# zhaoyuhsin/Edge-Guided-Near-Eye-Image-Analysis-for-Head-Mounted-Displays

Hardware: AMD Instinct MI355X
Metric: eye-frames/sec (320x240): inference edge+seg (value), +fit, exact fp32, and train fwd+bwd at 1 MI355X (higher is better)
Workload: dtype f32 tensors; inference products split into f16 hi/lo pairs (3 f16 MFMAs per product, 22-bit significand), f32 accumulate (`exact_fp32`: every product on the f32 MFMA); `train`: bf16 storage, f32 accumulate, f32 master weights (and an f32-storage leg)

## Files before the change

edge-guided-near-eye-image-analysis-for-head-mounted-displays_amd/_lib.py:

```python
import ctypes as C
import os

_HERE = os.path.dirname(os.path.abspath(__file__))
LIB_PATH = os.environ.get("EGNE_LIB") or os.path.join(_HERE, "csrc", "libegne_hip.so")

MAXSEG, MAXGROUP = 8, 3
ACT_NONE, ACT_RELU, ACT_LEAKY = 0, 1, 2

c_fp = C.c_void_p


class Seg(C.Structure):
    _fields_ = [("ptr", c_fp), ("pix_stride", C.c_int64), ("ch_off", C.c_int32), ("Cp", C.c_int32),
                ("scale", c_fp), ("shift", c_fp), ("act_in", C.c_int32), ("presplit", C.c_int32)]


class ConvDesc(C.Structure):
    _fields_ = [("B", C.c_int32), ("H", C.c_int32), ("W", C.c_int32), ("Ho", C.c_int32), ("Wo", C.c_int32),
                ("kh", C.c_int32), ("kw", C.c_int32), ("stride", C.c_int32),
                ("pad_h", C.c_int32), ("pad_w", C.c_int32), ("pad_mode", C.c_int32),
                ("ngroups", C.c_int32), ("dil", C.c_int32 * MAXGROUP),
                ("nseg", C.c_int32), ("seg", Seg * MAXSEG),
                ("Ktot", C.c_int32), ("CoutP", C.c_int32),
                ("w", c_fp), ("bias", c_fp), ("act", C.c_int32),
                ("post_scale", c_fp), ("post_shift", c_fp),
                ("residual", c_fp), ("res_pix_stride", C.c_int64), ("res_ch_off", C.c_int32),
                ("out", c_fp), ("out_pix_stride", C.c_int64), ("out_ch_off", C.c_int32),
                ("Cout_store", C.c_int32),
                ("stats_ws", c_fp), ("stats_nchunk", C.c_int32),
                ("pool_out", c_fp), ("pool_pix_stride", C.c_int64), ("pool_ch_off", C.c_int32),
                ("dyn_scale", C.c_void_p), ("absmax_out", C.c_void_p), ("dtype", C.c_int32),
                ("out_split", C.c_int32), ("out_split_scale", C.c_float), ("ovf_flag", C.c_void_p), ("f16_products", C.c_int32),
                ("mask_y", C.c_void_p), ("mask_pix_stride", C.c_int64), ("mask_ch_off", C.c_int32), ("mask_act", C.c_int32), ("mask_sums", C.c_void_p)]


class Dst(C.Structure):
    _fields_ = [("out", C.c_void_p), ("out_pix_stride", C.c_int64), ("out_ch_off", C.c_int32), ("C", C.c_int32), ("CoutP", C.c_int32),
                ("wfrag", C.c_void_p), ("residual", C.c_void_p), ("res_pix_stride", C.c_int64), ("res_ch_off", C.c_int32),
                ("mask_y", C.c_void_p), ("mask_pix_stride", C.c_int64), ("mask_ch_off", C.c_int32), ("act", C.c_int32),
                ("sums", C.c_void_p), ("res_pixels", C.c_int64)]


MAXDST = 6


class ConvQuery(C.Structure):
    _fields_ = [("dtype", C.c_int32), ("B", C.c_int32), ("H", C.c_int32), ("W", C.c_int32),
                ("kh", C.c_int32), ("kw", C.c_int32), ("stride", C.c_int32), ("pad_h", C.c_int32), ("pad_w", C.c_int32), ("pad_mode", C.c_int32),
                ("ngroups", C.c_int32), ("dil", C.c_int32 * MAXGROUP), ("nseg", C.c_int32),
                ("seg_C", C.c_int32 * MAXSEG), ("seg_Cp", C.c_int32 * MAXSEG), ("seg_ch_off", C.c_int32 * MAXSEG), ("seg_pix_stride", C.c_int64 * MAXSEG),
                ("seg_affine", C.c_int32 * MAXSEG), ("seg_planar", C.c_int32), ("seg_presplit", C.c_int32),
                ("Cout", C.c_int32), ("Cout_store", C.c_int32), ("dst_Cp", C.c_int32), ("dst_ch_off", C.c_int32), ("dst_pix_stride", C.c_int64),
                ("act", C.c_int32), ("has_post", C.c_int32), ("has_residual", C.c_int32), ("res_pix_stride", C.c_int64), ("res_ch_off", C.c_int32),
                ("split", C.c_int32), ("split1", C.c_int32), ("split_c4", C.c_int32), ("train", C.c_int32), ("dyn_scales", C.c_int32),
                ("is_dgrad", C.c_int32), ("want_stats", C.c_int32), ("want_pool", C.c_int32), ("pool_Cp", C.c_int32), ("pool_pix_stride", C.c_int64),
                ("want_scores", C.c_int32), ("up_add", C.c_int32), ("narrow_bf16_ok", C.c_int32), ("f16_products", C.c_int32), ("f16_storage", C.c_int32)]


class ConvChoice(C.Structure):
    _fields_ = [("kind", C.c_int32), ("name", C.c_char * 32), ("tail_frames", C.c_int32), ("fused_stats", C.c_int32), ("fused_pool", C.c_int32),
                ("small_ws_floats", C.c_int64)]


class BdcnTailDesc(C.Structure):
    _fields_ = [("B", C.c_int32), ("H", C.c_int32), ("W", C.c_int32),
                ("s", c_fp * 5), ("s1", c_fp * 5), ("h", C.c_int32 * 5), ("w", C.c_int32 * 5),
                ("stride", C.c_int32 * 5), ("crop", C.c_int32 * 5), ("up", c_fp * 5),
                ("fuse_w", c_fp), ("fuse_b", c_fp), ("out", c_fp * 11), ("edge_thres", C.c_int32)]


class LossDesc(C.Structure):
    _fields_ = [("B", C.c_int32), ("H", C.c_int32), ("W", C.c_int32),
                ("logits", c_fp), ("pix_stride", C.c_int64), ("ch_off", C.c_int32),
                ("target", c_fp), ("spatWts", c_fp), ("distMap", c_fp), ("cond", c_fp),
                ("pupil_center", c_fp), ("elNorm", c_fp), ("elOut", c_fp), ("alpha", C.c_float),
                ("grid_x", c_fp), ("grid_y", c_fp),
                ("partials", c_fp), ("out_terms", c_fp), ("pred_c", c_fp), ("elPred", c_fp),
                ("mask", c_fp), ("op_nchw", c_fp), ("coef", c_fp), ("dtype", C.c_int32),
                ("g_op_nchw", c_fp), ("g_pred_c", c_fp), ("g_elOut_up", c_fp)]


i32, i64, f32, vp = C.c_int32, C.c_int64, C.c_float, C.c_void_p
SIGNATURES = {
    "egne_conv2d_fwd": (i32, [C.POINTER(ConvDesc), vp]),
    "egne_pack_conv_weight": (i32, [vp, i32, i32, i32, i32, vp, i32, i32, vp, vp]),
    "egne_pack_conv_weight_frag": (i32, [vp, i32, i32, i32, i32, vp, i32, i32, vp, vp]),
    "egne_conv3x3_halo_supported": (i32, [C.POINTER(ConvDesc)]),
    "egne_conv3x3_halo_fwd": (i32, [C.POINTER(ConvDesc), vp]),
    "egne_conv3x3_smallcin_fwd": (i32, [C.POINTER(ConvDesc), vp, vp]),
    "egne_pack_conv_weight_f16x2": (i32, [vp, i32, i32, i32, i32, i32, i32, f32, vp, vp, vp]),
    "egne_conv2d_f16x3_fwd": (i32, [C.POINTER(ConvDesc), vp, vp, f32, f32, vp]),
    "egne_conv2d_f16x3_small_workspace_floats": (i64, [C.POINTER(ConvDesc)]),
    "egne_conv2d_f16x3_small_fwd": (i32, [C.POINTER(ConvDesc), vp, vp, f32, f32, vp, i64, vp]),
    "egne_pack_conv_weight_f16frag": (i32, [vp, i32, i32, i32, i32, i32, i32, f32, vp, vp, vp]),
    "egne_conv3x3_halo_f16_fwd": (i32, [C.POINTER(ConvDesc), vp, vp, f32, f32, vp]),
    "egne_conv1x1_3x3_fused_f16_fwd": (i32, [C.POINTER(ConvDesc), C.POINTER(ConvDesc), vp, vp, f32, f32, vp, vp, f32, f32, vp]),
    "egne_conv3x3c4_3x3_fused_f16_fwd": (i32, [C.POINTER(ConvDesc), C.POINTER(ConvDesc), vp, vp, f32, f32, vp, vp, f32, f32, vp]),
    "egne_msblock_dil_scores_f16_fwd": (i32, [C.POINTER(ConvDesc), vp, vp, f32, f32, vp, vp, vp, vp, i32, vp]),
    "egne_msblock_dil_f16_fwd": (i32, [C.POINTER(ConvDesc), vp, vp, f32, f32, vp]),
    "egne_conv3x3_rs_f16_fwd": (i32, [C.POINTER(ConvDesc), vp, vp, f32, f32, vp]),
    "egne_conv3x3_rw_f16_fwd": (i32, [C.POINTER(ConvDesc), vp, vp, f32, f32, vp]),
    "egne_conv1x1_pool2_f16x3_fwd": (i32, [C.POINTER(ConvDesc), vp, vp, f32, f32, vp]),
    "egne_conv1x1_f16x3_fwd": (i32, [C.POINTER(ConvDesc), vp, vp, f32, f32, vp]),
    "egne_dist_maps_workspace_bytes": (i64, [i32, i32, i32, i32]),
    "egne_dist_maps": (i32, [vp, i32, i32, i32, i32, vp, vp, vp]),
    "egne_zscore": (i32, [vp, vp, i32, i32, vp]),
    "egne_spatial_weights": (i32, [vp, i32, i32, i32, vp, vp]),
    "egne_eval_prep_workspace_bytes": (i64, [i32, i32, i32, i32, i32]),
    "egne_eval_prep": (i32, [vp, i32, i32, i32, i32, i32, i32, i32, vp, vp, vp, vp, i32, i32, vp, vp, vp, vp]),
    "egne_eval_render": (i32, [vp, i32, i32, i32, i32, i32, vp, vp, vp, i32, i32, C.c_double, i32, vp, vp, vp, vp, vp]),
    "egne_deepvog_loss_workspace_floats": (i64, [i32, i32, i32]),
    "egne_deepvog_loss_fwd": (i32, [vp, i64, i32, vp, vp, vp, i32, i32, i32, vp, vp, vp, vp, vp, vp]),
    "egne_deepvog_loss_bwd": (i32, [vp, i64, i32, vp, vp, vp, i32, i32, i32, vp, vp, vp, vp, i64, i32, vp]),
    "egne_affine_act": (i32, [vp, i64, i32, vp, i64, i32, i32, i64, vp, vp, i32, vp]),
    "egne_augment": (i32, [vp, vp, vp, vp, vp, vp, vp, vp, i32, i32, i32, vp]),
    "egne_augment_cv": (i32, [vp, vp, vp, vp, vp, vp, vp, vp, vp, vp, i32, i32, i32, vp]),
    "egne_conv3x3_smallcin_f16_fwd": (i32, [C.POINTER(ConvDesc), vp, vp, f32, f32, vp]),
    "egne_pack_conv3x3_c4_weight_f16": (i32, [vp, i32, i32, i32, f32, vp, vp, vp]),
    "egne_conv1x1_ms_f16x3_fwd": (i32, [C.POINTER(ConvDesc), vp, vp, f32, f32, vp]),
    "egne_pack_conv1x1_weight_f16x2_map": (i32, [vp, i32, i32, vp, i32, i32, f32, vp, vp, vp]),
    "egne_conv2d_f16x3_big_fwd": (i32, [C.POINTER(ConvDesc), vp, f32, f32, vp]),
    "egne_pack_conv_weight_f16img": (i32, [vp, i32, i32, i32, i32, i32, i32, f32, vp, vp]),
    "egne_conv2d_f16_big1_fwd": (i32, [C.POINTER(ConvDesc), vp, f32, f32, vp]),
    "egne_conv2d_f16_big1_supported": (i32, [C.POINTER(ConvDesc)]),
    "egne_pack_conv_weight_f16img1": (i32, [vp, i32, i32, i32, i32, i32, i32, f32, vp, vp]),
    "egne_pack_conv1x1_weight_f16": (i32, [vp, i32, i32, vp, i32, i32, f32, vp, vp, vp]),
    "egne_absmax": (i32, [vp, i64, i32, i32, i64, vp, vp]),
    "egne_absmax_f16": (i32, [vp, i64, i32, i32, i64, vp, vp]),
    "egne_norm_stats_workspace_bytes": (i64, [i32, i32, i32, i32]),
    "egne_norm_stats": (i32, [vp, i64, i32, i32, i32, i32, i32, f32, vp, vp, vp, vp, vp, vp]),
    "egne_norm_stats_finish": (i32, [vp, i32, i32, i32, i32, f32, vp, vp, vp]),
    "egne_norm_stats_finish_moments": (i32, [vp, i32, i32, i32, i32, f32, vp, vp, vp, vp, vp]),
    "egne_affine_inplace": (i32, [vp, i64, i32, i32, i64, vp, vp, vp]),
    "egne_affine": (i32, [vp, i64, i32, vp, i64, i32, i32, i64, vp, vp, vp]),
    "egne_avgpool2": (i32, [vp, i64, i32, vp, i64, i32, i32, i32, i32, i32, vp]),
    "egne_norm_act_pool2": (i32, [vp, i64, i32, vp, vp, i32, vp, i64, i32, i32, i32, i32, i32, vp]),
    "egne_maxpool2": (i32, [vp, i64, i32, vp, i64, i32, i32, i32, i32, i32, i32, i32, i32, vp]),
    "egne_maxpool2_f16": (i32, [vp, i64, i32, vp, i64, i32, i32, i32, i32, i32, i32, i32, i32, vp]),
    "egne_maxpool2_split": (i32, [vp, i64, i32, vp, i64, i32, i32, i32, i32, i32, i32, i32, i32, vp]),
    "egne_upsample2x": (i32, [vp, i64, i32, vp, i64, i32, i32, i32, i32, i32, vp]),
    "egne_upsample2x_nearest": (i32, [vp, i64, i32, vp, i64, i32, i32, i32, i32, i32, vp]),
    "egne_upsample2x_nearest_bwd": (i32, [vp, i64, i32, vp, i64, i32, i32, i32, i32, i32, vp]),
    "egne_nchw_to_nhwc": (i32, [vp, i32, i32, i32, i32, vp, i64, i32, i32, vp]),
    "egne_nhwc_to_nchw": (i32, [vp, i64, i32, i32, i32, i32, i32, vp, vp]),
    "egne_bdcn_stage_scores": (i32, [C.POINTER(vp), i32, i64, i64, vp, vp, vp, vp, vp, vp, vp, vp, vp]),
    "egne_bdcn_tail": (i32, [C.POINTER(BdcnTailDesc), vp]),
    "egne_loss_workspace_floats": (i64, [i32, i32, i32]),
    "egne_loss_fwd": (i32, [C.POINTER(LossDesc), vp]),
    "egne_ellipse_head_act": (i32, [vp, i32, i32, vp]),
    "egne_selu_inplace": (i32, [vp, i64, vp]),
    "egne_spatial_mean": (i32, [vp, i64, i32, i32, i32, i32, vp, vp]),
    "egne_softmax3": (i32, [vp, i64, i32, vp, i64, i32, i32, i64, vp]),
    "egne_adain": (i32, [vp, i64, i32, i32, vp, vp, i64, i32, vp, i64, i32, i32, i32, f32, vp]),
    "egne_conf_loss": (i32, [vp, i32, vp, i32, i32, i32, f32, vp, vp]),
    "egne_loss_bwd": (i32, [C.POINTER(LossDesc), vp, vp, i64, i32, vp, vp]),
    "egne_act_bwd_bias_workspace_bytes": (i64, [i64, i32]),
    "egne_act_bwd_bias": (i32, [vp, i64, i32, vp, i64, i32, i32, i32, i64, vp, i32, i32, vp, vp]),
    "egne_act_bwd_bias_absmax": (i32, [vp, i64, i32, vp, i64, i32, i32, i32, i64, vp, i32, i32, vp, vp, vp]),
    "egne_act_norm_bwd": (i32, [vp, i64, i32, vp, i64, i32, i32, vp, vp, vp, i64, i32, vp, i64, i32, i32, i32, i32, i32, i32, vp, vp, vp, i32, vp, i32, vp]),
    "egne_bn_act_bwd": (i32, [vp, i64, i32, i32, vp, vp, vp, vp, i64, i32, i32, i32, i32, i32, vp, i64, i32, vp, vp, vp, vp, i32, vp, i32, vp, vp]),
    "egne_zero_many": (i32, [vp, i32, i64, vp]),
    "egne_pair_bias_bwd_workspace_bytes": (i64, [i32, i32]),
    "egne_pair_bias_bwd": (i32, [vp, i64, i32, i32, i32, i32, i32, vp, vp, i32, i32, vp, vp, vp, vp]),
    "egne_norm_bwd_workspace_bytes": (i64, [i32, i32, i32, i32]),
    "egne_norm_pool2_bwd": (i32, [vp, i64, i32, vp, vp, vp, i64, i32, i32, i32, i32, i32, i32, vp, i64, i32, i32, vp, vp, vp]),
    "egne_norm_bwd_store": (i32, [vp, i64, i32, vp, vp, vp, vp, i64, i32, i32, i32, i32, i32, i32, vp, i64, i32, vp, vp, vp,
                                  i32, vp, vp]),
    "egne_norm_bwd": (i32, [vp, i64, i32, vp, vp, vp, vp, i64, i32, i32, i32, i32, i32, i32, vp, i64, i32, vp, vp, vp,
                            i32, vp, vp]),
    "egne_avgpool2_bwd": (i32, [vp, i64, i32, vp, i64, i32, i32, i32, i32, i32, vp]),
    "egne_upsample2x_bwd": (i32, [vp, i64, i32, vp, i64, i32, i32, i32, i32, i32, vp]),
    "egne_upsample2x_bwd_store": (i32, [vp, i64, i32, vp, i64, i32, i32, i32, i32, i32, vp]),
    "egne_ellipse_head_act_bwd": (i32, [vp, vp, i32, i32, vp]),
    "egne_selu_bwd": (i32, [vp, vp, i64, vp]),
    "egne_softmax3_bwd": (i32, [vp, i64, i32, vp, i64, i32, vp, i64, i32, i64, vp]),
    "egne_adain_bwd": (i32, [vp, i64, i32, i32, vp, i64, i32, vp, i64, i32, vp, i64, i32, vp, vp, i64, i32, i32, i32, f32, vp]),
    "egne_reflect_pad_bwd": (i32, [vp, i64, i32, i32, i32, vp, i64, i32, i32, i32, i32, i32, vp]),
    "egne_spatial_mean_bwd": (i32, [vp, i32, vp, i64, i32, i32, i32, i32, vp]),
    "egne_conf_loss_bwd": (i32, [vp, i32, vp, i32, i32, i32, vp, vp, i32, vp]),
    "egne_conv2d_wgrad_splits": (i32, [C.POINTER(ConvDesc)]),
    "egne_conv2d_wgrad_workspace_bytes": (i64, [C.POINTER(ConvDesc)]),
    "egne_conv2d_wgrad": (i32, [C.POINTER(ConvDesc), vp, i64, i32, i32, i32, vp, C.POINTER(vp), vp, vp]),
    "egne_conv2d_wgrad_f16": (i32, [C.POINTER(ConvDesc), vp, i64, i32, vp, i32, i32, vp, C.POINTER(vp), vp, vp]),
    "egne_pack_conv_weight_dgrad": (i32, [vp, i32, i32, i32, i32, i32, i32, i32, i32, i32, vp, vp]),
    "egne_ellipse_fit": (i32, [vp, i32, vp, vp, i32, i32, i32, vp, vp, vp, vp, vp, vp]),
    "egne_ellipse_init_from_pred": (i32, [vp, i32, i32, i32, vp, vp, vp, vp]),
# ... 63 lines not shown
```

edge-guided-near-eye-image-analysis-for-head-mounted-displays_amd/csrc/common.h:

```cpp
#pragma once
#include <hip/hip_runtime.h>
#include <cstdarg>
#include <cstdio>
#include <mutex>
#include <unordered_map>
#include "../../include/egne_hip.h"

static __device__ __attribute__((aligned(256), used)) float egne_zero_page[64] = {0};

typedef __bf16 egne_bf16;
typedef float egne_f32x4 __attribute__((ext_vector_type(4)));
typedef __bf16 egne_bf16x4 __attribute__((ext_vector_type(4)));
typedef __bf16 egne_bf16x8 __attribute__((ext_vector_type(8)));

__device__ __forceinline__ egne_f32x4 ld4(const float* p) { return *(const egne_f32x4*)p; }
__device__ __forceinline__ egne_f32x4 ld4(const egne_bf16* p) { return __builtin_convertvector(*(const egne_bf16x4*)p, egne_f32x4); }
__device__ __forceinline__ void st4(float* p, egne_f32x4 v) { *(egne_f32x4*)p = v; }
__device__ __forceinline__ void st4(egne_bf16* p, egne_f32x4 v) { *(egne_bf16x4*)p = __builtin_convertvector(v, egne_bf16x4); }
__device__ __forceinline__ float ld1(const float* p) { return *p; }
__device__ __forceinline__ float ld1(const egne_bf16* p) { return (float)*p; }
__device__ __forceinline__ void st1(float* p, float v) { *p = v; }
__device__ __forceinline__ void st1(egne_bf16* p, float v) { *p = (egne_bf16)v; }
template <typename T> struct egne_vt { static constexpr int N = 4; };
template <> struct egne_vt<egne_bf16> { static constexpr int N = 8; };
// ... 20 lines not shown
  *(egne_bf16x8*)p = egne_bf16x8{l[0], l[1], l[2], l[3], h[0], h[1], h[2], h[3]};
}
typedef unsigned egne_u32x4 __attribute__((ext_vector_type(4)));
template <typename T> __device__ __forceinline__ egne_u32x4 ldraw(const T* p) { return *(const egne_u32x4*)p; }
__device__ __forceinline__ egne_fv<4> unpackv(const float*, egne_u32x4 w) {
  return egne_fv<4>{{__builtin_bit_cast(float, w[0]), __builtin_bit_cast(float, w[1]), __builtin_bit_cast(float, w[2]), __builtin_bit_cast(float, w[3])}};
}
__device__ __forceinline__ egne_fv<8> unpackv(const egne_bf16*, egne_u32x4 w) {
  egne_fv<8> r;
#pragma unroll
  for (int i = 0; i < 4; ++i) {
    r.v[2 * i] = __builtin_bit_cast(float, w[i] << 16);
    r.v[2 * i + 1] = __builtin_bit_cast(float, w[i] & 0xffff0000u);
  }
  return r;
}
template <int N> __device__ __forceinline__ egne_fv<N> ldf(const float* p) {
  egne_fv<N> r;
#pragma unroll
  for (int i = 0; i < N; i += 4) { const egne_f32x4 t = *(const egne_f32x4*)(p + i); r.v[i] = t[0]; r.v[i + 1] = t[1]; r.v[i + 2] = t[2]; r.v[i + 3] = t[3]; }
  return r;
}
template <int N> __device__ __forceinline__ egne_fv<N> fv_fill(float x) {
  egne_fv<N> r;
#pragma unroll
  for (int i = 0; i < N; ++i) r.v[i] = x;
  return r;
}
template <typename T> __device__ __forceinline__ const T* zero_page() { return (const T*)egne_zero_page; }

#ifdef EGNE_NO_OVF_CHECK
__device__ __forceinline__ bool egne_nonfinite(float) { return false; }
__device__ __forceinline__ bool egne_nonfinite64(double) { return false; }
#else
__device__ __forceinline__ bool egne_nonfinite(float v) { return __builtin_amdgcn_classf(v, 0x207); }
__device__ __forceinline__ bool egne_nonfinite64(double v) { return !__builtin_isfinite(v); }
#endif
__device__ __forceinline__ bool egne_ovf_row(int y, int H) { return y % 3 == 1 || y == H - 1; }
__device__ __forceinline__ void egne_ovf_commit(bool bad, unsigned* flag) {
  if (flag && bad) atomicOr(flag, 1u);
}

namespace egne {

char* err_buf();

inline int fail(int code, const char* fmt, ...) {
  va_list ap;
  va_start(ap, fmt);
  vsnprintf(err_buf(), 512, fmt, ap);
  va_end(ap);
  return code;
}

inline bool fp32_storage(const egne_conv_desc& d) {
  for (int i = 0; i < d.nseg && i < EGNE_MAXSEG; ++i)
    if (d.seg[i].presplit != 0) return false;
  return d.out_split == 0;
}

inline int check_launch(const char* what) {
  hipError_t e = hipGetLastError();
  if (e != hipSuccess) return fail(EGNE_ERR_LAUNCH, "%s: %s", what, hipGetErrorString(e));
  return EGNE_OK;
}

inline bool raise_lds(const void* kern, size_t bytes) {
  static std::mutex mu;
  static std::unordered_map<const void*, size_t> have;
  std::lock_guard<std::mutex> g(mu);
  auto it = have.find(kern);
  if (it != have.end() && it->second >= bytes) return true;
  if (hipFuncSetAttribute(kern, hipFuncAttributeMaxDynamicSharedMemorySize, (int)bytes) != hipSuccess) {
    (void)hipGetLastError();
    return false;
  }
  have[kern] = bytes;
  return true;
}

#define EGNE_REQUIRE(cond, ...) \
  do { if (!(cond)) return ::egne::fail(EGNE_ERR_ARG, __VA_ARGS__); } while (0)

bool halo3_supported(const egne_conv_desc& d);
int halo3_launch(const egne_conv_desc& d, hipStream_t st);

bool wgrad_halo_supported(const egne_conv_desc& d, long long gzs);
int wgrad_halo_splits(const egne_conv_desc& d);
int wgrad_halo_launch(const egne_conv_desc& d, const float* gz, long long gzs, int gzo, float* ws, hipStream_t st);
int wgrad_halo_f16_launch(const egne_conv_desc& d, const float* gz, long long gzs, int gzo, const unsigned* gz_dyn, float* ws, hipStream_t st);

bool wgrad3x3_bf16_supported(const egne_conv_desc& d, long long gzs);
int wgrad3x3_bf16_splits(const egne_conv_desc& d);
int wgrad3x3_bf16_launch(const egne_conv_desc& d, const egne_bf16* gz, long long gzs, int gzo, float* ws, hipStream_t st);
bool wgrad1x1_bf16_supported(const egne_conv_desc& d, long long gzs);
int wgrad1x1_bf16_splits(const egne_conv_desc& d);
int wgrad1x1_bf16_launch(const egne_conv_desc& d, const egne_bf16* gz, long long gzs, int gzo, float* ws, hipStream_t st);

int msdil_ps_launch(const egne_conv_desc& d, const void* fhi, const void* flo, float a_scale, float w_scale, const float* score_w,
                    const float* score_c, float* s0, float* s1, int accumulate, hipStream_t st);

bool msdil1_wanted(const egne_conv_desc& d);
int msdil1_launch(const egne_conv_desc& d, const void* fhi, float a_scale, float w_scale, const float* score_w, const float* score_c,
                  float* s0, float* s1, int accumulate, hipStream_t st);

inline int cdiv(long long a, long long b) { return (int)((a + b - 1) / b); }

}
```

edge-guided-near-eye-image-analysis-for-head-mounted-displays_amd/csrc/conv1x1_f16.hip:

```cpp
#include "common.h"
#include "split_f16.h"

typedef float f32x16 __attribute__((ext_vector_type(16)));
typedef float f32x4 __attribute__((ext_vector_type(4)));
typedef float f32x2 __attribute__((ext_vector_type(2)));
typedef _Float16 h8 __attribute__((ext_vector_type(8)));
typedef _Float16 h2 __attribute__((ext_vector_type(2)));
typedef unsigned u32x4 __attribute__((ext_vector_type(4)));

namespace {

constexpr unsigned OOB = 0x80000000u;

__device__ __forceinline__ __amdgpu_buffer_rsrc_t make_rsrc(const void* base, unsigned bytes) {
  return __builtin_amdgcn_make_buffer_rsrc(const_cast<void*>(base), 0, (int)bytes, 0x00020000);
}

__device__ __forceinline__ void split8(const u32x4 a, const u32x4 b, float s, h8& hi, h8& lo) {
  const f32x4 va = __builtin_bit_cast(f32x4, a), vb = __builtin_bit_cast(f32x4, b);
  const float x[8] = {va[0], va[1], va[2], va[3], vb[0], vb[1], vb[2], vb[3]};
#pragma unroll
  for (int q = 0; q < 4; ++q) {
    h2 h, l;
    egne::split2(x[2 * q], x[2 * q + 1], s, h, l);
// ... 367 lines not shown
  EGNE_REQUIRE(lds <= 80 * 1024, "conv1x1_f16: K = %d groups of 16 does not fit the LDS weight image", G);
  static bool once = [] {
    return hipFuncSetAttribute((const void*)conv1x1_f16x3_kernel<1>, hipFuncAttributeMaxDynamicSharedMemorySize, 80 * 1024) == hipSuccess &&
           hipFuncSetAttribute((const void*)conv1x1_f16x3_kernel<2>, hipFuncAttributeMaxDynamicSharedMemorySize, 80 * 1024) == hipSuccess;
  }();
  if (!once) return egne::fail(EGNE_ERR_LAUNCH, "conv1x1_f16: cannot raise the dynamic LDS limit");
  const int ny = d.CoutP / (32 * TN);
  long long gx = (nb + 3) / 4;
  const long long cap = 256 * 8;
  if (gx > cap) gx = cap;
  const float os = 1.0f / (a_scale * w_scale);
  hipStream_t st = (hipStream_t)stream;
  if (up) {
    const size_t lds_up = lds + (size_t)4 * 18 * (32 * TN + 8) * sizeof(float);
    EGNE_REQUIRE(lds_up <= 80 * 1024, "conv1x1_f16: K = %d groups of 16 leaves no room for the addend patches", G);
    static bool once_up = [] {
      return hipFuncSetAttribute((const void*)conv1x1_f16x3_kernel<1, true>, hipFuncAttributeMaxDynamicSharedMemorySize, 80 * 1024) == hipSuccess &&
             hipFuncSetAttribute((const void*)conv1x1_f16x3_kernel<2, true>, hipFuncAttributeMaxDynamicSharedMemorySize, 80 * 1024) == hipSuccess;
    }();
    if (!once_up) return egne::fail(EGNE_ERR_LAUNCH, "conv1x1_f16: cannot raise the dynamic LDS limit");
    if (TN == 1)
      hipLaunchKernelGGL((conv1x1_f16x3_kernel<1, true>), dim3((unsigned)gx, ny), dim3(256), lds_up, st, d, (const _Float16*)fhi, (const _Float16*)flo,
                         a_scale, os, G, M, (int)nb);
    else
      hipLaunchKernelGGL((conv1x1_f16x3_kernel<2, true>), dim3((unsigned)gx, ny), dim3(256), lds_up, st, d, (const _Float16*)fhi, (const _Float16*)flo,
                         a_scale, os, G, M, (int)nb);
  } else if (TN == 1)
    hipLaunchKernelGGL((conv1x1_f16x3_kernel<1>), dim3((unsigned)gx, ny), dim3(256), lds, st, d, (const _Float16*)fhi, (const _Float16*)flo,
                       a_scale, os, G, M, (int)nb);
  else
    hipLaunchKernelGGL((conv1x1_f16x3_kernel<2>), dim3((unsigned)gx, ny), dim3(256), lds, st, d, (const _Float16*)fhi, (const _Float16*)flo,
                       a_scale, os, G, M, (int)nb);
  return egne::check_launch("egne_conv1x1_f16x3_fwd");
}

extern "C" int egne_conv1x1_pool2_f16x3_fwd(const egne_conv_desc* dp, const void* fhi, const void* flo, float a_scale, float w_scale,
                                            void* stream) {
  EGNE_REQUIRE(dp && fhi && flo, "conv1x1_pool2_f16: null pointer");
  const egne_conv_desc& d = *dp;
  EGNE_REQUIRE(egne::fp32_storage(d), "conv1x1_f16: split-pair / f16 storage (presplit, out_split) is not known here");
  EGNE_REQUIRE(d.kh == 1 && d.kw == 1 && d.stride == 1 && d.pad_h == 0 && d.pad_w == 0 && d.ngroups == 1 && d.Ho == d.H / 2 && d.Wo == d.W / 2 &&
               d.Ho > 0 && d.Wo > 0 && d.nseg >= 1 && d.nseg <= EGNE_MAXSEG && !d.residual && !d.post_scale, "conv1x1_pool2_f16: unsupported descriptor");
  EGNE_REQUIRE(d.CoutP % 32 == 0 && d.CoutP <= 96 && d.Cout_store <= d.CoutP && d.Cout_store % 4 == 0 && d.out &&
               ((uintptr_t)d.out & 15) == 0 && d.out_pix_stride % 4 == 0 && d.out_ch_off % 4 == 0 &&
               d.out_ch_off + d.Cout_store <= d.out_pix_stride && (!d.bias || ((uintptr_t)d.bias & 15) == 0), "conv1x1_pool2_f16: output");
  int G = 0;
  for (int s = 0; s < d.nseg; ++s) {
    const egne_seg& g = d.seg[s];
    EGNE_REQUIRE(g.ptr && g.scale && g.shift && ((uintptr_t)g.scale & 15) == 0 && ((uintptr_t)g.shift & 15) == 0 && g.Cp % 8 == 0 &&
                 g.ch_off % 4 == 0 && g.pix_stride % 4 == 0 && ((uintptr_t)g.ptr & 15) == 0 && g.ch_off + g.Cp <= g.pix_stride &&
                 (long long)d.H * d.W * g.pix_stride * 8 < (1ll << 31), "conv1x1_pool2_f16: slice %d", s);
    G += (g.Cp + 15) / 16;
  }
  EGNE_REQUIRE(d.out_pix_stride * 128 < (1ll << 31) && ((uintptr_t)fhi & 15) == 0 && ((uintptr_t)flo & 15) == 0 && a_scale > 0.f && w_scale > 0.f,
               "conv1x1_pool2_f16: strides / weights / scales");
  const long long M = (long long)d.B * d.Ho * d.Wo;
  const long long nb = (M + 31) / 32;
  EGNE_REQUIRE(nb < (1ll << 31), "conv1x1_pool2_f16: too many pixels");
  const int TN = d.CoutP / 32;
  const int bpf = (d.Ho * d.Wo + 31) / 32;
  EGNE_REQUIRE(!d.stats_ws || (((uintptr_t)d.stats_ws & 15) == 0 && d.stats_nchunk >= 1 && d.stats_nchunk <= bpf &&
                               (long long)(d.stats_nchunk - 1) * ((bpf + d.stats_nchunk - 1) / d.stats_nchunk) < bpf &&
                               (long long)d.B * d.stats_nchunk < (1ll << 31)),
               "conv1x1_pool2_f16: stats_ws needs 1 <= stats_nchunk <= %d blocks per frame, no empty chunk", bpf);
  const size_t lds = (size_t)G * TN * 2 * 64 * 8 * sizeof(_Float16) + (d.stats_ws ? (size_t)4 * 32 * 36 * sizeof(float) : 0);
  EGNE_REQUIRE(lds <= 80 * 1024, "conv1x1_pool2_f16: K = %d groups of 16 does not fit the LDS weight image", G);
  static bool once = [] {
    return hipFuncSetAttribute((const void*)conv1x1_pool_f16x3_kernel<1>, hipFuncAttributeMaxDynamicSharedMemorySize, 80 * 1024) == hipSuccess &&
           hipFuncSetAttribute((const void*)conv1x1_pool_f16x3_kernel<2>, hipFuncAttributeMaxDynamicSharedMemorySize, 80 * 1024) == hipSuccess &&
           hipFuncSetAttribute((const void*)conv1x1_pool_f16x3_kernel<3>, hipFuncAttributeMaxDynamicSharedMemorySize, 80 * 1024) == hipSuccess &&
           hipFuncSetAttribute((const void*)conv1x1_pool_f16x3_kernel<1, true>, hipFuncAttributeMaxDynamicSharedMemorySize, 80 * 1024) == hipSuccess &&
           hipFuncSetAttribute((const void*)conv1x1_pool_f16x3_kernel<2, true>, hipFuncAttributeMaxDynamicSharedMemorySize, 80 * 1024) == hipSuccess &&
           hipFuncSetAttribute((const void*)conv1x1_pool_f16x3_kernel<3, true>, hipFuncAttributeMaxDynamicSharedMemorySize, 80 * 1024) == hipSuccess;
  }();
  if (!once) return egne::fail(EGNE_ERR_LAUNCH, "conv1x1_pool2_f16: cannot raise the dynamic LDS limit");
  const int ny = 1;
  const long long nu = d.stats_ws ? (long long)d.B * d.stats_nchunk : nb;
  long long gx = (nu + 3) / 4;
  const long long cap = 256 * 8;
  if (gx > cap) gx = cap;
  const float os = 1.0f / (a_scale * w_scale);
  hipStream_t st = (hipStream_t)stream;
  const dim3 grid((unsigned)gx, (unsigned)ny);
  const _Float16* h = (const _Float16*)fhi;
  const _Float16* l = (const _Float16*)flo;
  if (d.stats_ws) {
    if (TN == 1) hipLaunchKernelGGL((conv1x1_pool_f16x3_kernel<1, true>), grid, dim3(256), lds, st, d, h, l, a_scale, os, G, M, (int)nu);
    else if (TN == 2) hipLaunchKernelGGL((conv1x1_pool_f16x3_kernel<2, true>), grid, dim3(256), lds, st, d, h, l, a_scale, os, G, M, (int)nu);
    else hipLaunchKernelGGL((conv1x1_pool_f16x3_kernel<3, true>), grid, dim3(256), lds, st, d, h, l, a_scale, os, G, M, (int)nu);
  } else if (TN == 1) hipLaunchKernelGGL((conv1x1_pool_f16x3_kernel<1>), grid, dim3(256), lds, st, d, h, l, a_scale, os, G, M, (int)nu);
  else if (TN == 2) hipLaunchKernelGGL((conv1x1_pool_f16x3_kernel<2>), grid, dim3(256), lds, st, d, h, l, a_scale, os, G, M, (int)nu);
  else hipLaunchKernelGGL((conv1x1_pool_f16x3_kernel<3>), grid, dim3(256), lds, st, d, h, l, a_scale, os, G, M, (int)nu);
  return egne::check_launch("egne_conv1x1_pool2_f16x3_fwd");
}
```

include/egne_hip.h:

```cpp
#ifndef EGNE_HIP_H
#define EGNE_HIP_H

#include <stdint.h>

#ifdef __cplusplus
extern "C" {
#endif

#define EGNE_MAXSEG 8
#define EGNE_MAXGROUP 3

typedef enum {
  EGNE_OK = 0,
  EGNE_ERR_ARG = -1,
  EGNE_ERR_LAUNCH = -2,
  EGNE_ERR_NODEVICE = -3
} egne_status;

typedef enum { EGNE_ACT_NONE = 0, EGNE_ACT_RELU = 1, EGNE_ACT_LEAKY = 2 } egne_act;

typedef struct {
  const float* ptr;
  int64_t pix_stride;
  int32_t ch_off;
// ... 1 lines not shown
  const float* scale;
  const float* shift;
  int32_t act_in;
  int32_t presplit;
} egne_seg;

typedef struct {
  int32_t B, H, W;
  int32_t Ho, Wo;
  int32_t kh, kw, stride;
  int32_t pad_h, pad_w;
  int32_t pad_mode;
  int32_t ngroups;
  int32_t dil[EGNE_MAXGROUP];
  int32_t nseg;
  egne_seg seg[EGNE_MAXSEG];
  int32_t Ktot;
  int32_t CoutP;
  const float* w;
  const float* bias;
  int32_t act;
  const float* post_scale;
  const float* post_shift;
  const float* residual;
  int64_t res_pix_stride;
  int32_t res_ch_off;
  float* out;
  int64_t out_pix_stride;
  int32_t out_ch_off;
  int32_t Cout_store;
  double* stats_ws;
  int32_t stats_nchunk;
  float* pool_out;
  int64_t pool_pix_stride;
  int32_t pool_ch_off;
  const uint32_t* dyn_scale;
  uint32_t* absmax_out;
  int32_t dtype;
  int32_t out_split;
  float out_split_scale;
  uint32_t* ovf_flag;
  int32_t f16_products;
  const void* mask_y; int64_t mask_pix_stride; int32_t mask_ch_off; int32_t mask_act;
  float* mask_sums;
} egne_conv_desc;

int egne_conv2d_fwd(const egne_conv_desc* d, void* stream);
int egne_conv3x3_bf16_sum_rows(void);

int egne_conv3x3_halo_supported(const egne_conv_desc* d);
int egne_conv3x3_halo_fwd(const egne_conv_desc* d, void* stream);
int egne_pack_conv_weight_frag(const float* w_oihw, int Cout, int Cin, int kh, int kw,
                               const int32_t* kinv, int CoutP, int Ktot, float* w_packed, void* stream);

int egne_pack_conv_weight_f16x2(const float* w_oihw, int Cout, int Cin, int kh, int kw, int CoutP, int Ktot,
                                float wscale, void* whi, void* wlo, void* stream);
int egne_conv2d_f16x3_fwd(const egne_conv_desc* d, const void* whi, const void* wlo, float a_scale,
                          float w_scale, void* stream);
int64_t egne_conv2d_f16x3_small_workspace_floats(const egne_conv_desc* d);
int egne_conv2d_f16x3_small_fwd(const egne_conv_desc* d, const void* whi, const void* wlo, float a_scale, float w_scale,
                                float* ws, int64_t ws_floats, void* stream);

int egne_pack_conv_weight_f16img(const float* w_oihw, int Cout, int Cin, int kh, int kw, int BN, int Ktot, float wscale,
                                 void* wimg, void* stream);
int egne_conv2d_f16x3_big_fwd(const egne_conv_desc* d, const void* wimg, float a_scale, float w_scale, void* stream);
int egne_pack_conv_weight_f16img1(const float* w_oihw, int Cout, int Cin, int kh, int kw, int BN, int Ktot, float wscale,
                                  void* wimg, void* stream);
int egne_conv2d_f16_big1_supported(const egne_conv_desc* d);
int egne_conv2d_f16_big1_fwd(const egne_conv_desc* d, const void* wimg, float a_scale, float w_scale, void* stream);

int egne_pack_conv_weight_f16frag(const float* w_oihw, int Cout, int Cin, int kh, int kw, int CoutP, int Ktot,
                                  float wscale, void* fhi, void* flo, void* stream);
int egne_conv3x3_halo_f16_fwd(const egne_conv_desc* d, const void* fhi, const void* flo, float a_scale,
                              float w_scale, void* stream);

int egne_msblock_dil_f16_fwd(const egne_conv_desc* d, const void* fhi, const void* flo, float a_scale, float w_scale,
                             void* stream);
int egne_msblock_dil_scores_f16_fwd(const egne_conv_desc* d, const void* fhi, const void* flo, float a_scale, float w_scale,
                                    const float* score_w, const float* score_c, float* s0, float* s1, int accumulate,
                                    void* stream);

int egne_conv1x1_pool2_f16x3_fwd(const egne_conv_desc* d, const void* fhi, const void* flo, float a_scale, float w_scale,
                                 void* stream);

int egne_conv3x3_rs_f16_fwd(const egne_conv_desc* d, const void* fhi, const void* flo, float a_scale, float w_scale,
                            void* stream);

int egne_conv3x3_rw_f16_fwd(const egne_conv_desc* d, const void* fhi, const void* flo, float a_scale, float w_scale,
                            void* stream);

int egne_pack_conv1x1_weight_f16(const float* w_oihw, int Cout, int Cin, const int32_t* kmap, int G, int CoutP,
                                 float wscale, void* fhi, void* flo, void* stream);
int egne_conv1x1_f16x3_fwd(const egne_conv_desc* d, const void* fhi, const void* flo, float a_scale,
                           float w_scale, void* stream);

int egne_conv1x1_3x3_fused_f16_fwd(const egne_conv_desc* d1, const egne_conv_desc* d2, const void* w1hi, const void* w1lo,
                                   float a1, float w1_scale, const void* f2hi, const void* f2lo, float a2, float w2_scale,
                                   void* stream);

int egne_conv3x3c4_3x3_fused_f16_fwd(const egne_conv_desc* d1, const egne_conv_desc* d2, const void* c4hi, const void* c4lo,
                                     float a1, float w1_scale, const void* f2hi, const void* f2lo, float a2, float w2_scale,
                                     void* stream);

int egne_pack_conv1x1_weight_f16x2_map(const float* w_oihw, int Cout, int Cin, const int32_t* kmap, int CoutP, int Ktot,
                                       float wscale, void* whi, void* wlo, void* stream);
int egne_conv1x1_ms_f16x3_fwd(const egne_conv_desc* d, const void* whi, const void* wlo, float a_scale,
                              float w_scale, void* stream);

int egne_conv3x3_smallcin_fwd(const egne_conv_desc* d, const float* w40, void* stream);

int egne_pack_conv3x3_c4_weight_f16(const float* w_oihw, int Cout, int Cin, int CoutP, float wscale, void* fhi, void* flo,
                                    void* stream);
int egne_conv3x3_smallcin_f16_fwd(const egne_conv_desc* d, const void* fhi, const void* flo, float a_scale,
                                  float w_scale, void* stream);

int egne_pack_conv_weight(const float* w_oihw, int Cout, int Cin, int kh, int kw,
                          const int32_t* kinv, int CoutP, int Ktot, float* w_packed, void* stream);

int egne_absmax(const float* x, int64_t pix_stride, int ch_off, int Cp, int64_t npix, void* out_bits, void* stream);
int egne_absmax_f16(const void* x, int64_t pix_stride, int ch_off, int Cp, int64_t npix, void* out_bits, void* stream);

int64_t egne_norm_stats_workspace_bytes(int B, int HW, int Cp, int per_sample);
int egne_norm_stats(const float* x, int64_t pix_stride, int ch_off, int Cp, int B, int HW,
                    int per_sample, float eps, float* scale, float* shift,
                    float* mean_out, float* var_out, void* ws, void* stream);

int egne_norm_stats_finish(const void* ws, int Cp, int B, int nchunk, int HW, float eps, float* scale, float* shift,
                           void* stream);
int egne_norm_stats_finish_moments(const void* ws, int Cp, int B, int nchunk, int HW, float eps, float* scale, float* shift,
                                   float* mean_out, float* var_out, void* stream);

int egne_affine_inplace(float* x, int64_t pix_stride, int ch_off, int Cp, int64_t npix,
                        const float* scale, const float* shift, void* stream);

int egne_affine(const float* x, int64_t xs, int xo, float* y, int64_t ys, int yo, int Cp, int64_t npix,
                const float* scale, const float* shift, void* stream);

int egne_avgpool2(const float* x, int64_t xs, int xo, float* y, int64_t ys, int yo,
                  int B, int H, int W, int Cp, void* stream);

int egne_norm_act_pool2(const float* x, int64_t xs, int xo, const float* scale, const float* shift, int act,
                        float* y, int64_t ys, int yo, int B, int H, int W, int Cp, void* stream);

int egne_maxpool2(const float* x, int64_t xs, int xo, float* y, int64_t ys, int yo,
                  int B, int H, int W, int Ho, int Wo, int stride, int Cp, void* stream);
int egne_maxpool2_f16(const void* x, int64_t xs, int xo, void* y, int64_t ys, int yo, int B, int H, int W, int Ho, int Wo, int stride,
                      int Cp, void* stream);

int egne_maxpool2_split(const void* x, int64_t xs, int xo, void* y, int64_t ys, int yo, int B, int H, int W, int Ho, int Wo, int stride,
                        int Cp, void* stream);

int egne_upsample2x(const float* x, int64_t xs, int xo, float* y, int64_t ys, int yo,
                    int B, int H, int W, int Cp, void* stream);

int egne_nchw_to_nhwc(const float* x, int B, int C, int H, int W, float* y, int64_t ys, int yo,
                      int Cp, void* stream);
int egne_nhwc_to_nchw(const float* x, int64_t xs, int xo, int B, int C, int H, int W, float* y,
                      void* stream);

int egne_bdcn_stage_scores(const float* const* ms, int nblk, int64_t ms_pix_stride, int64_t npix,
                           const float* wd, const float* bd, const float* ws, const float* bs,
                           const float* ws1, const float* bs1, float* s, float* s1, void* stream);

typedef struct {
  int32_t B, H, W;
  const float* s[5];
// ... 317 lines not shown
```

Baseline: 2134.

## Stage conv1x1+pool inputs through async buffer-to-LDS DMA ring

Adds a new conv1x1 avgpool2 f16x3 kernel that streams the input patches, plus the per-channel scale and shift, directly into a per-wave multi-stage LDS ring using buffer_load_lds. A swizzled slot layout avoids bank conflicts, and the pooling, affine and activation steps read from LDS while the next stage's loads are in flight. The goal is to hide global-memory latency behind the MFMA work. It is on by default when the LDS budget fits, and the cost is a large LDS footprint, lower occupancy and hand-managed vmcnt waits.

Measured after the change: 2108. 0.988x the previous value.

```diff
diff --git a/edge-guided-near-eye-image-analysis-for-head-mounted-displays_amd/_lib.py b/edge-guided-near-eye-image-analysis-for-head-mounted-displays_amd/_lib.py
--- a/edge-guided-near-eye-image-analysis-for-head-mounted-displays_amd/_lib.py
+++ b/edge-guided-near-eye-image-analysis-for-head-mounted-displays_amd/_lib.py
@@ -102,6 +102,8 @@
     "egne_conv3x3_rw_f16_fwd": (i32, [C.POINTER(ConvDesc), vp, vp, f32, f32, vp]),
     "egne_conv1x1_pool2_f16x3_fwd": (i32, [C.POINTER(ConvDesc), vp, vp, f32, f32, vp]),
     "egne_conv1x1_f16x3_fwd": (i32, [C.POINTER(ConvDesc), vp, vp, f32, f32, vp]),
+    "egne_conv1x1_dma_slot": (i32, [i32, i32, i32, i32]),
+    "egne_conv1x1_dma_lds_bytes": (i64, [i32, i32, i32, i32]),
     "egne_dist_maps_workspace_bytes": (i64, [i32, i32, i32, i32]),
     "egne_dist_maps": (i32, [vp, i32, i32, i32, i32, vp, vp, vp]),
     "egne_zscore": (i32, [vp, vp, i32, i32, vp]),
diff --git a/edge-guided-near-eye-image-analysis-for-head-mounted-displays_amd/csrc/common.h b/edge-guided-near-eye-image-analysis-for-head-mounted-displays_amd/csrc/common.h
--- a/edge-guided-near-eye-image-analysis-for-head-mounted-displays_amd/csrc/common.h
+++ b/edge-guided-near-eye-image-analysis-for-head-mounted-displays_amd/csrc/common.h
@@ -126,6 +126,10 @@
 #define EGNE_REQUIRE(cond, ...) \
   do { if (!(cond)) return ::egne::fail(EGNE_ERR_ARG, __VA_ARGS__); } while (0)
 
+int conv1x1_pool_dma_gps(int G, int TN, bool stats);
+int conv1x1_pool_dma_launch(const egne_conv_desc& d, int gps, const void* fhi, const void* flo, float a_scale, float os, int G, long long M,
+                            long long nu, hipStream_t st);
+
 bool halo3_supported(const egne_conv_desc& d);
 int halo3_launch(const egne_conv_desc& d, hipStream_t st);
 
diff --git a/edge-guided-near-eye-image-analysis-for-head-mounted-displays_amd/csrc/conv1x1_dma_f16.hip b/edge-guided-near-eye-image-analysis-for-head-mounted-displays_amd/csrc/conv1x1_dma_f16.hip
--- /dev/null
+++ b/edge-guided-near-eye-image-analysis-for-head-mounted-displays_amd/csrc/conv1x1_dma_f16.hip
@@ -0,0 +1,339 @@
+#include "common.h"
+#include "conv1x1_dma_slot.h"
+#include "split_f16.h"
+
+typedef float f32x16 __attribute__((ext_vector_type(16)));
+typedef float f32x4 __attribute__((ext_vector_type(4)));
+typedef _Float16 h8 __attribute__((ext_vector_type(8)));
+typedef _Float16 h2 __attribute__((ext_vector_type(2)));
+typedef unsigned u32x4 __attribute__((ext_vector_type(4)));
+typedef __attribute__((address_space(3))) void* lds_ptr;
+
+namespace {
+
+using namespace egne::dma1x1;
+
+constexpr unsigned OOB = 0x80000000u;
+
+__device__ __forceinline__ __amdgpu_buffer_rsrc_t make_rsrc(const void* base, unsigned bytes) {
+  return __builtin_amdgcn_make_buffer_rsrc(const_cast<void*>(base), 0, (int)bytes, 0x00020000);
+}
+
+template <int N>
+__device__ __forceinline__ void wait_vm() {
+  asm volatile("s_waitcnt vmcnt(%0)" ::"n"(N) : "memory");
+}
+
+__device__ __forceinline__ void split8(const u32x4 a, const u32x4 b, float s, h8& hi, h8& lo) {
+  const f32x4 va = __builtin_bit_cast(f32x4, a), vb = __builtin_bit_cast(f32x4, b);
+  const float x[8] = {va[0], va[1], va[2], va[3], vb[0], vb[1], vb[2], vb[3]};
+#pragma unroll
+  for (int q = 0; q < 4; ++q) {
+    h2 h, l;
+    egne::split2(x[2 * q], x[2 * q + 1], s, h, l);
+    hi[2 * q] = h[0]; hi[2 * q + 1] = h[1];
+    lo[2 * q] = l[0]; lo[2 * q + 1] = l[1];
+  }
+}
+
+template <int TN, bool STATS, int GPS>
+__global__ __launch_bounds__(256) void conv1x1_pool_dma_kernel(const egne_conv_desc p, const _Float16* __restrict__ fhi,
+                                                               const _Float16* __restrict__ flo, float a_scale, float out_scale,
+                                                               int G, long long M, int nblocks) {
+  constexpr int DATA_PIECES = data_pieces(GPS), AUX_BYTES = aux_bytes(GPS), STAGE_BYTES = stage_bytes(GPS), STAGES = stages(GPS);
+  constexpr int ND = DATA_PIECES + 2;
+  constexpr int CH = chunks(GPS), PPX = 16 * GPS, PPI = 64 / PPX, NV = 16 / PPI;
+  extern __shared__ __attribute__((aligned(1024))) char lds[];
+  _Float16* const wl = (_Float16*)lds;
+  const int tid = threadIdx.x, lane = tid & 63;
+  const int wave = __builtin_amdgcn_readfirstlane(tid >> 6);
+  const int li = lane & 31, kq = lane >> 5;
+  const int NT = p.CoutP >> 5;
+  for (int it = tid; it < G * TN * 2 * 64; it += 256) {
+    const int l = it & 63, hl = (it >> 6) & 1;
+    const int tn = (it >> 7) % TN, g = (it >> 7) / TN;
+    const _Float16* src = (hl ? flo : fhi) + (((long long)g * NT + tn) * 64 + l) * 8;
+    *(u32x4*)&wl[(long long)it * 8] = *(const u32x4*)src;
+  }
+  float* const lbias = (float*)(lds + (long long)G * TN * 2048);
+  for (int n = tid; n < 32 * TN; n += 256) lbias[n] = (p.bias && n < p.Cout_store) ? p.bias[n] : 0.f;
+  __syncthreads();
+
+  const float slope = p.act == EGNE_ACT_RELU ? 0.f : (p.act == EGNE_ACT_LEAKY ? 0.01f : 1.f);
+  const int H = p.H, W = p.W, Wp = p.Wo, hwp = p.Ho * p.Wo;
+  const float s4 = 0.25f * a_scale;
+  constexpr bool stats = STATS;
+  const int bpf = (hwp + 31) >> 5, cb = stats ? (bpf + p.stats_nchunk - 1) / p.stats_nchunk : 1;
+  constexpr int PP = 36;
+  [[maybe_unused]] float* const patch = (float*)(lbias + 128) + wave * (16 * PP);
+  [[maybe_unused]] const int rd = (lane >> 5) * PP + (lane & 31);
+  char* const ring = (char*)(lbias + 128) + (stats ? PATCH_BYTES : 0) + wave * (STAGES * STAGE_BYTES);
+
+  auto unit_range = [&](int u, long long& mfirst, long long& mend) {
+    mfirst = (long long)u * 32; mend = M;
+    if (stats) {
+      const int fb = u / p.stats_nchunk, ck = u - fb * p.stats_nchunk;
+      mfirst = (long long)fb * hwp + (long long)ck * cb * 32;
+      mend = (long long)(fb + 1) * hwp;
+    }
+    if (mend > mfirst + (long long)cb * 32) mend = mfirst + (long long)cb * 32;
+  };
+  auto locate = [&](long long m0, long long mend, int& b0, bool& valid, int& fr, int& pin) {
+    const int rows = mend - m0 < 32 ? (int)(mend - m0) : 32;
+    b0 = (int)(m0 / hwp);
+    const int rr = (int)(m0 - (long long)b0 * hwp) + li;
+    valid = li < rows;
+    fr = valid ? rr / hwp : 0;
+    const int r = rr - fr * hwp;
+    const int yp = valid ? r / Wp : 0, xp = valid ? r - yp * Wp : 0;
+    pin = (fr * H + 2 * yp) * W + 2 * xp;
+  };
+
+  const int lp = lane / PPX, lq = lane % PPX;
+  int tapoff[NV], cq[NV];
+#pragma unroll
+  for (int r = 0; r < NV; ++r) {
+    const int q = lq ^ (r * PPI + lp), t = q / CH;
+    cq[r] = q % CH;
+    tapoff[r] = (t >> 1) * W + (t & 1);
+  }
+  int iu = blockIdx.x * 4 + wave, is = 0, igg = 0, in16 = 0, ib0 = 0;
+  long long im0 = 0, imend = 0;
+  bool ilive = iu < nblocks;
+  int pofs[DATA_PIECES];
+  auto enter_block = [&]() {
+    bool valid; int fr, pin;
+    locate(im0, imend, ib0, valid, fr, pin);
+    const int mine = valid ? pin : -1;
+#pragma unroll
+    for (int i = 0; i < DATA_PIECES; ++i) {
+      const int v = __shfl(mine, i * PPI + lp);
+      pofs[i] = v < 0 ? -1 : v + tapoff[i % NV];
+    }
+  };
+#pragma unroll
+  for (int i = 0; i < DATA_PIECES; ++i) pofs[i] = -1;
+  if (ilive) {
+    unit_range(iu, im0, imend);
+    enter_block();
+    in16 = (p.seg[0].Cp + 15) >> 4;
+  }
+  auto issue = [&](char* dst) {
+    asm volatile("" ::: "memory");
+    const egne_seg sg = p.seg[is];
+    const long long frame = (long long)H * W * sg.pix_stride;
+    const long long left = ((long long)p.B - ib0) * frame * 4;
+    const __amdgpu_buffer_rsrc_t rs = make_rsrc(sg.ptr + (long long)ib0 * frame, ilive ? (unsigned)(left < 2 * frame * 4 ? left : 2 * frame * 4) : 0u);
+    const unsigned affb = ilive ? (unsigned)((long long)p.B * sg.Cp * 4) : 0u;
+    const __amdgpu_buffer_rsrc_t rsc = make_rsrc(sg.scale, affb), rsh = make_rsrc(sg.shift, affb);
+    const int tail8 = (sg.Cp & 15) != 0 ? 1 : 0;
+    const int cend = (in16 - igg) * 4 - 2 * tail8;
+    const int ps4 = (int)sg.pix_stride * 4;
+    if (lane < 2 * CH) {
+      const int f = lane / CH, c = lane % CH;
+      const int off = c >= cend ? (int)OOB : (((ib0 + f) * sg.Cp + igg * 16 + 4 * c) * 4);
+      __builtin_amdgcn_raw_ptr_buffer_load_lds(rsc, (lds_ptr)dst, 16, off, 0, 0, 0);
+      __builtin_amdgcn_raw_ptr_buffer_load_lds(rsh, (lds_ptr)(dst + AUX_BYTES / 2), 16, off, 0, 0, 0);
+    }
+#pragma unroll
+    for (int i = 0; i < DATA_PIECES; ++i) {
+      const int c = cq[i % NV];
+      const int off = (pofs[i] < 0 || c >= cend) ? (int)OOB : pofs[i] * ps4 + (sg.ch_off + 4 * c) * 4;
+      __builtin_amdgcn_raw_ptr_buffer_load_lds(rs, (lds_ptr)(dst + AUX_BYTES + i * 1024), 16, off, igg * 64, 0, 0);
+    }
+    asm volatile("" ::: "memory");
+    if (ilive && (igg += GPS) >= in16) {
+      igg = 0;
+      if (++is == p.nseg) {
+        is = 0;
+        im0 += 32;
+        if (im0 >= imend) {
+          iu += gridDim.x * 4;
+          ilive = iu < nblocks;
+          if (ilive) unit_range(iu, im0, imend);
+        }
+        if (ilive) enter_block();
+      }
+      if (ilive) in16 = (p.seg[is].Cp + 15) >> 4;
+      else is = 0;
+    }
+  };
+#pragma unroll
+  for (int k = 0; k < STAGES; ++k) issue(ring + k * STAGE_BYTES);
+
+  int slot = 0, cool = 0;
+  const int key = li & 15;
+  for (int unit = blockIdx.x * 4 + wave; unit < nblocks; unit += gridDim.x * 4) {
+   long long mfirst, mend;
+   unit_range(unit, mfirst, mend);
+   [[maybe_unused]] double ssum[TN], qsum[TN];
+#pragma unroll
+   for (int tn = 0; tn < TN; ++tn) ssum[tn] = qsum[tn] = 0.;
+   for (long long m0 = mfirst; m0 < mend; m0 += 32) {
+    const long long rows = mend - m0 < 32 ? mend - m0 : 32;
+    int b0, fr, pin;
+    bool valid;
+    locate(m0, mend, b0, valid, fr, pin);
+    const int fro = (fr > 1 ? 1 : fr) * (AUX_BYTES / 4) + kq * 16;
+    f32x16 acc[TN];
+#pragma unroll
+    for (int tn = 0; tn < TN; ++tn) acc[tn] = (f32x16)(0.f);
+    int g = 0;
+    for (int s = 0; s < p.nseg; ++s) {
+      const egne_seg sg = p.seg[s];
+      const float slope_in = sg.act_in == EGNE_ACT_RELU ? 0.f : (sg.act_in == EGNE_ACT_LEAKY ? 0.01f : 1.f);
+      const int n16 = (sg.Cp + 15) >> 4;
+      for (int gg = 0; gg < n16; gg += GPS) {
+        if (cool > 0) { wait_vm<(STAGES - 1) * ND + 4 * TN>(); --cool; }
+        else wait_vm<(STAGES - 1) * ND>();
+        char* const st = ring + slot * STAGE_BYTES;
+        const char* dp = st + AUX_BYTES + li * (PPX * 16);
+        h8 ah[GPS], al[GPS];
+#pragma unroll
+        for (int u = 0; u < GPS; ++u) {
+          if (u == 0 || gg + u < n16) {
+            u32x4 xa[4], xb[4];
+#pragma unroll
+            for (int t = 0; t < 4; ++t) {
+              xa[t] = *(const u32x4*)(dp + (((t * CH + u * 4 + kq) ^ key) << 4));
+              xb[t] = *(const u32x4*)(dp + (((t * CH + u * 4 + kq + 2) ^ key) << 4));
+            }
+            const char* ap = st + fro + u * 64;
+            const f32x4 sca = *(const f32x4*)ap, scb = *(const f32x4*)(ap + 32);
+            const f32x4 sha = *(const f32x4*)(ap + AUX_BYTES / 2), shb = *(const f32x4*)(ap + AUX_BYTES / 2 + 32);
+            f32x4 sa = (f32x4)(0.f), sb = (f32x4)(0.f);
+#pragma unroll
+            for (int t = 0; t < 4; ++t) {
+              f32x4 va = __builtin_bit_cast(f32x4, xa[t]) * sca + sha, vb = __builtin_bit_cast(f32x4, xb[t]) * scb + shb;
+#pragma unroll
+              for (int e = 0; e < 4; ++e) { sa[e] += fmaxf(va[e], va[e] * slope_in); sb[e] += fmaxf(vb[e], vb[e] * slope_in); }
+            }
+            if (!valid) { sa = (f32x4)(0.f); sb = (f32x4)(0.f); }
+            split8(__builtin_bit_cast(u32x4, sa), __builtin_bit_cast(u32x4, sb), s4, ah[u], al[u]);
+          }
+        }
+        issue(st);
+        slot = slot == STAGES - 1 ? 0 : slot + 1;
+#pragma unroll
+        for (int u = 0; u < GPS; ++u) {
+          if (u == 0 || gg + u < n16) {
+            const _Float16* wp = wl + ((long long)(g + gg + u) * TN * 2 * 64 + lane) * 8;
+#pragma unroll
+            for (int tn = 0; tn < TN; ++tn) {
+              const h8 wh = *(const h8*)(wp + (tn * 2 + 0) * 512), wo = *(const h8*)(wp + (tn * 2 + 1) * 512);
+              acc[tn] = __builtin_amdgcn_mfma_f32_32x32x16_f16(wh, al[u], acc[tn], 0, 0, 0);
+              acc[tn] = __builtin_amdgcn_mfma_f32_32x32x16_f16(wo, ah[u], acc[tn], 0, 0, 0);
+              acc[tn] = __builtin_amdgcn_mfma_f32_32x32x16_f16(wh, ah[u], acc[tn], 0, 0, 0);
+            }
+          }
+        }
+      }
+      g += n16;
+    }
+    const __amdgpu_buffer_rsrc_t ro = make_rsrc(p.out + m0 * p.out_pix_stride, (unsigned)(rows * p.out_pix_stride * 4));
+    bool bad = false;
+#pragma unroll
+    for (int tn = 0; tn < TN; ++tn) {
+      [[maybe_unused]] f32x4 sv[4];
+#pragma unroll
+      for (int j = 0; j < 4; ++j) {
+        const int n = tn * 32 + 8 * j + 4 * kq;
+        const f32x4 bv = *(const f32x4*)(lbias + n);
+        f32x4 v;
+#pragma unroll
+        for (int e = 0; e < 4; ++e) {
+          const float t = acc[tn][4 * j + e] * out_scale + bv[e];
+          v[e] = fmaxf(t, t * slope);
+        }
+        if (tn == 0 && j == 0) bad |= egne_nonfinite(v[0]);
+        const int off = n < p.Cout_store ? (li * (int)p.out_pix_stride + p.out_ch_off + n) * 4 : (int)OOB;
+        __builtin_amdgcn_raw_buffer_store_b128(__builtin_bit_cast(u32x4, v), ro, off, 0, 0);
+        if constexpr (stats) sv[j] = valid ? v : (f32x4)(0.f);
+      }
+      if constexpr (stats) {
+        double s_ = ssum[tn], q_ = qsum[tn];
+#pragma unroll
+        for (int hf = 0; hf < 2; ++hf) {
+          if ((li >> 4) == hf) {
+#pragma unroll
+            for (int j = 0; j < 4; ++j) *(f32x4*)&patch[(li & 15) * PP + 8 * j + 4 * kq] = sv[j];
+          }
+          asm volatile("s_waitcnt lgkmcnt(0)" ::: "memory");
+#pragma unroll
+          for (int i = 0; i < 8; ++i) {
+            const double x = (double)patch[i * 2 * PP + rd];
+            s_ += x; q_ += x * x;
+          }
+          asm volatile("s_waitcnt lgkmcnt(0)" ::: "memory");
+        }
+        ssum[tn] = s_; qsum[tn] = q_;
+      }
+    }
+    egne_ovf_commit(bad, p.ovf_flag);
+    cool = STAGES;
+   }
+   if constexpr (stats) {
+#pragma unroll
+     for (int tn = 0; tn < TN; ++tn) {
+       const double s_ = ssum[tn] + __shfl_xor(ssum[tn], 32), q_ = qsum[tn] + __shfl_xor(qsum[tn], 32);
+       const int n = tn * 32 + lane;
+       if (lane < 32 && n < p.Cout_store)
+         ((double2*)p.stats_ws)[(long long)unit * p.Cout_store + n] = make_double2(s_, q_);
+     }
+   }
+  }
+  wait_vm<0>();
+}
+
+template <int TN, bool STATS, int GPS>
+int launch(const egne_conv_desc& d, const _Float16* h, const _Float16* l, float a_scale, float os, int G, long long M, long long nu, size_t lds,
+           hipStream_t st) {
+  if (!egne::raise_lds((const void*)conv1x1_pool_dma_kernel<TN, STATS, GPS>, lds))
+    return egne::fail(EGNE_ERR_LAUNCH, "conv1x1_pool2_f16 (staged): cannot raise the dynamic LDS limit to %zu", lds);
+  long long gx = (nu + 3) / 4;
+  if (gx > 256 * 8) gx = 256 * 8;
+  hipLaunchKernelGGL((conv1x1_pool_dma_kernel<TN, STATS, GPS>), dim3((unsigned)gx), dim3(256), lds, st, d, h, l, a_scale, os, G, M, (int)nu);
+  return egne::check_launch("egne_conv1x1_pool2_f16x3_fwd (staged)");
+}
+
+}
+
+namespace egne {
+
+int conv1x1_pool_dma_gps(int G, int TN, bool stats) {
+  const char* e = getenv("EGNE_CONV1X1_DMA");
+  const int want = e ? atoi(e) : 2;
+  if (want <= 0) return 0;
+  if (want >= 2 && dma1x1::lds_bytes(G, TN, stats, 2) <= dma1x1::LDS_LIMIT) return 2;
+  return dma1x1::lds_bytes(G, TN, stats, 1) <= dma1x1::LDS_LIMIT ? 1 : 0;
+}
+
+int conv1x1_pool_dma_launch(const egne_conv_desc& d, int gps, const void* fhi, const void* flo, float a_scale, float os, int G, long long M,
+                            long long nu, hipStream_t st) {
+  const int TN = d.CoutP / 32;
+  const bool stats = d.stats_ws != nullptr;
+  const size_t lds = (size_t)dma1x1::lds_bytes(G, TN, stats, gps);
+  const _Float16* h = (const _Float16*)fhi;
+  const _Float16* l = (const _Float16*)flo;
+#define EGNE_DMA_CASE(TNV, SV, GV) \
+  if (TN == TNV && stats == SV && gps == GV) return launch<TNV, SV, GV>(d, h, l, a_scale, os, G, M, nu, lds, st);
+  EGNE_DMA_CASE(1, true, 1) EGNE_DMA_CASE(2, true, 1) EGNE_DMA_CASE(3, true, 1)
+  EGNE_DMA_CASE(1, false, 1) EGNE_DMA_CASE(2, false, 1) EGNE_DMA_CASE(3, false, 1)
+  EGNE_DMA_CASE(1, true, 2) EGNE_DMA_CASE(2, true, 2) EGNE_DMA_CASE(3, true, 2)
+  EGNE_DMA_CASE(1, false, 2) EGNE_DMA_CASE(2, false, 2) EGNE_DMA_CASE(3, false, 2)
+#undef EGNE_DMA_CASE
+  return fail(EGNE_ERR_ARG, "conv1x1_pool2_f16 (staged): no instance for TN %d, %d groups per stage", TN, gps);
+}
+
+}
+
+extern "C" int egne_conv1x1_dma_slot(int gps, int pixel, int tap, int chunk) {
+  if (gps < 1 || gps > 2 || pixel < 0 || pixel >= egne::dma1x1::PIXELS || tap < 0 || tap >= egne::dma1x1::TAPS || chunk < 0 ||
+      chunk >= egne::dma1x1::chunks(gps))
+    return -1;
+  return egne::dma1x1::slot(gps, pixel, tap, chunk);
+}
+
+extern "C" long long egne_conv1x1_dma_lds_bytes(int G, int TN, int stats, int gps) {
+  return gps < 1 || gps > 2 ? -1 : egne::dma1x1::lds_bytes(G, TN, stats != 0, gps);
+}
diff --git a/edge-guided-near-eye-image-analysis-for-head-mounted-displays_amd/csrc/conv1x1_dma_slot.h b/edge-guided-near-eye-image-analysis-for-head-mounted-displays_amd/csrc/conv1x1_dma_slot.h
--- /dev/null
+++ b/edge-guided-near-eye-image-analysis-for-head-mounted-displays_amd/csrc/conv1x1_dma_slot.h
@@ -0,0 +1,24 @@
+#pragma once
+
+namespace egne {
+namespace dma1x1 {
+
+constexpr int PIXELS = 32, TAPS = 4, WAVES = 4;
+constexpr int LDS_LIMIT = 160 * 1024;
+constexpr int PATCH_BYTES = WAVES * 16 * 36 * 4;
+
+constexpr int chunks(int gps) { return 4 * gps; }
+constexpr int data_pieces(int gps) { return PIXELS * TAPS * chunks(gps) / 64; }
+constexpr int data_bytes(int gps) { return PIXELS * TAPS * chunks(gps) * 16; }
+constexpr int aux_bytes(int gps) { return 256 * gps; }
+constexpr int stage_bytes(int gps) { return aux_bytes(gps) + data_bytes(gps); }
+constexpr int stages(int gps) { return gps == 1 ? 3 : 2; }
+
+constexpr int slot(int gps, int pixel, int tap, int chunk) { return pixel * 16 * gps + ((tap * chunks(gps) + chunk) ^ (pixel & 15)); }
+
+constexpr long long lds_bytes(int G, int TN, bool stats, int gps) {
+  return (long long)G * TN * 2048 + 512 + (stats ? PATCH_BYTES : 0) + (long long)WAVES * stages(gps) * stage_bytes(gps);
+}
+
+}
+}
diff --git a/edge-guided-near-eye-image-analysis-for-head-mounted-displays_amd/csrc/conv1x1_f16.hip b/edge-guided-near-eye-image-analysis-for-head-mounted-displays_amd/csrc/conv1x1_f16.hip
--- a/edge-guided-near-eye-image-analysis-for-head-mounted-displays_amd/csrc/conv1x1_f16.hip
+++ b/edge-guided-near-eye-image-analysis-for-head-mounted-displays_amd/csrc/conv1x1_f16.hip
@@ -473,6 +473,7 @@
   const float os = 1.0f / (a_scale * w_scale);
   hipStream_t st = (hipStream_t)stream;
   const dim3 grid((unsigned)gx, (unsigned)ny);
+  if (const int gps = egne::conv1x1_pool_dma_gps(G, TN, d.stats_ws != nullptr)) return egne::conv1x1_pool_dma_launch(d, gps, fhi, flo, a_scale, os, G, M, nu, st);
   const _Float16* h = (const _Float16*)fhi;
   const _Float16* l = (const _Float16*)flo;
   if (d.stats_ws) {
diff --git a/include/egne_hip.h b/include/egne_hip.h
--- a/include/egne_hip.h
+++ b/include/egne_hip.h
@@ -107,6 +107,9 @@
 
 int egne_conv1x1_pool2_f16x3_fwd(const egne_conv_desc* d, const void* fhi, const void* flo, float a_scale, float w_scale,
                                  void* stream);
+
+int egne_conv1x1_dma_slot(int gps, int pixel, int tap, int chunk);
+long long egne_conv1x1_dma_lds_bytes(int G, int TN, int stats, int gps);
 
 int egne_conv3x3_rs_f16_fwd(const egne_conv_desc* d, const void* fhi, const void* flo, float a_scale, float w_scale,
                             void* stream);
```
